# mahbhlddnhakkh/yuv-manipulations-2

Measured on AMD Instinct MI355X. Metric: megapixels/sec DCT compress+decompress, 4K IYUV; achieved HBM GB/s vs peak, higher is better.
Workload: dtype u8/int16 (fp32 transform)

## Files before the change

### yuv-manipulations-2_amd/csrc/k_huff_decode.hip

```cpp
#include "codec_common.hpp"
#include "coef_xform.h"
#include "downscale.h"
#include "huff_common.hpp"
#include "idct_scaled.h"
#include "jpeg_export.h"
#include "k1_store.hpp"
#include "k_metric.hpp"
#include "k_stream.hpp"
#include "requant.h"
#include "xform_common.hpp"

namespace myyuv_gpu {

namespace {

constexpr uint32_t kStageQuads = 320;
constexpr uint32_t kZeroBit = kStageQuads * 128u;
constexpr uint32_t kGposQuads = 8 * 64 * 4 / 16;

#ifndef MYYUV_K5_GROUP
#define MYYUV_K5_GROUP 2
#endif
#ifndef MYYUV_K5_FORMS
#define MYYUV_K5_FORMS 1
// ... 434 lines not shown

__global__ __launch_bounds__(64, MYYUV_K5_WAVES) void k_decode_idct(const uint8_t* __restrict__ in,
                                                   const uint32_t* __restrict__ in_size,
                                                   uint32_t cap,
                                                   const StreamDesc* __restrict__ desc,
                                                   const uint32_t* __restrict__ local_off,
                                                   const uint32_t* __restrict__ tile_pre,
                                                   FrameGeom G, uint32_t tiles_p0,
                                                   uint32_t tiles_p1, const QTables* __restrict__ qt,
                                                   uint4* __restrict__ coef,
                                                   uint8_t* __restrict__ frame,
                                                   unsigned long long* __restrict__ err) {
  static_assert(sizeof(uint4) * kStageQuads >= sizeof(float) * xf::kXfTile16, "the tile over the stage");
  __shared__ uint4 stq[kStageQuads + 1 + kGposQuads];
  __shared__ float sq[64];
  __shared__ uint16_t s_blk[64];
  const uint32_t lane = threadIdx.x;
  if (lane == 0) stq[kStageQuads] = make_uint4(0u, 0u, 0u, 0u);
  {
    const uint32_t t = blockIdx.x;
    const int p = t >= tiles_p0 ? (t >= tiles_p0 + tiles_p1 ? 2 : 1) : 0;
    __builtin_amdgcn_global_load_lds((const void*)&qt->q[p][lane], (__attribute__((address_space(3))) void*)sq, 4,
                                     0, 0);
  }
#ifdef MYYUV_STAMPS
  DStamps dst;
  DStamps* ds = &dst;
  dst.prev = __builtin_amdgcn_s_memtime();
#pragma unroll
  for (int k = 0; k < 8; k++) dst.acc[k] = k == 7 ? 1u : 0u;
#else
  DStamps* ds = nullptr;
#endif
  DecodeGroup D;
  uint32_t nw[32];
#pragma unroll
  for (int w = 0; w < 32; w++) nw[w] = 0;
  bool direct;
  if (!decode_group(in, in_size, cap, desc, local_off, tile_pre, G, tiles_p0, tiles_p1, coef, err, stq, D, nw,
                    direct, ds))
    return;
  DSTAMP(4);
  if (D.live && direct) {
#pragma unroll
    for (int c = 0; c < 8; c++) {
      const uint4 v = coef[coef_quad(D.gbase + D.g, c)];
      nw[4 * c] = v.x;
      nw[4 * c + 1] = v.y;
      nw[4 * c + 2] = v.z;
      nw[4 * c + 3] = v.w;
    }
  }
  const int p = D.p;
  xf::Unit U;
  U.p = p;
  U.cum = G.cum[p];
  U.nb = G.cum[p + 1] - G.cum[p];
  U.poff = p == 0 ? G.poff[0] : (p == 1 ? G.poff[1] : G.poff[2]);
  U.pw = p == 0 ? G.pw[0] : (p == 1 ? G.pw[1] : G.pw[2]);
  U.bw = p == 0 ? G.bw[0] : (p == 1 ? G.bw[1] : G.bw[2]);
  U.bmag = p == 0 ? G.bmag[0] : (p == 1 ? G.bmag[1] : G.bmag[2]);
  U.local0 = 0;
  uint8_t* fr = frame + (size_t)D.f * G.fbytes;
  uint32_t acc = nw[0] & 0xFFFF0000u;
#pragma unroll
  for (int w = 1; w < 32; w++) acc |= nw[w];
  const bool isdc = D.live && acc == 0u;
  if (isdc) {
    const uint32_t v4 = dc_block_pixels((int16_t)nw[0], sq[0]);
    const uint2 row = make_uint2(v4, v4);
#pragma unroll
    for (uint32_t r = 0; r < 8; r++) {
      const uint32_t off = xf::block_row_offset(U, D.g - U.cum, r);
      *reinterpret_cast<uint2*>(fr + off) = row;
    }
  }
  const uint64_t rest = __ballot(D.live && !isdc);
  const uint32_t nrest = (uint32_t)__popcll(rest);
  const uint32_t rrank = __builtin_amdgcn_mbcnt_hi((uint32_t)(rest >> 32), __builtin_amdgcn_mbcnt_lo((uint32_t)rest, 0u));
  if (D.live && !isdc) s_blk[rrank] = (uint16_t)lane;
  float* tile = reinterpret_cast<float*>(stq);
#pragma unroll 1
  for (uint32_t base = 0; base < nrest;) {
    const bool wide = nrest - base > 8u;
    const uint32_t span = wide ? 16u : 8u, stride = wide ? (uint32_t)xf::kTile : (uint32_t)xf::kTile8;
    const uint32_t s = rrank - base;
    if (D.live && !isdc && rrank >= base && s < span) {
      uint4* img = reinterpret_cast<uint4*>(tile + s * stride + (wide ? xf::img_word(s) : 0u));
#pragma unroll
      for (int c = 0; c < 8; c++) img[c] = make_uint4(nw[4 * c], nw[4 * c + 1], nw[4 * c + 2], nw[4 * c + 3]);
    }
    if (lane < span && base + lane >= nrest) {
      uint4* img = reinterpret_cast<uint4*>(tile + lane * stride + (wide ? xf::img_word(lane) : 0u));
#pragma unroll
      for (int c = 0; c < 8; c++) img[c] = make_uint4(0u, 0u, 0u, 0u);
    }
    xf::wave_sync();
    if (wide) {
      const uint32_t q = lane & 3u, b = lane >> 2;
      uint2 w0, w1;
      xf::idct_rows(tile + b * xf::kTile, q, b, sq, w0, w1);
      if (base + b < nrest) {
        const uint32_t gl = D.g0 + s_blk[base + b];
        const uint32_t off = xf::block_row_offset(U, gl - U.cum, 2u * q);
        *reinterpret_cast<uint2*>(fr + off) = w0;
        *reinterpret_cast<uint2*>(fr + off + U.pw) = w1;
      }
    } else {
      const uint32_t r = lane & 7u, b = lane >> 3;
      float qc[8];
#pragma unroll
      for (int k = 0; k < 8; k++) qc[k] = sq[8 * k + r];
      const uint2 w = xf::idct_row8(tile + b * xf::kTile8, r, qc);
      if (base + b < nrest) {
        const uint32_t gl = D.g0 + s_blk[base + b];
        *reinterpret_cast<uint2*>(fr + xf::block_row_offset(U, gl - U.cum, r)) = w;
      }
    }
    xf::wave_sync();
    base += span;
  }
  DSTAMP(5);
#ifdef MYYUV_STAMPS
  const uint32_t wid = blockIdx.y * gridDim.x + blockIdx.x;
#pragma unroll
  for (int k = 0; k < 8; k++)
    if (lane == (uint32_t)k && wid < 65536) g_dec_wstamps[wid * 8 + k] = dst.acc[k];
#endif
}

constexpr uint32_t kSpanStageQuads = 288;
constexpr uint32_t kSpanZeroBit = kSpanStageQuads * 128u;
constexpr uint32_t kSpanGroups = kDecSpan / kWave;
static_assert(sizeof(uint4) * kSpanStageQuads >= sizeof(float) * xf::kXfTile16, "the tile over the stage");
static_assert(16 * (kSpanStageQuads - 1) >= 15 + 255, "a round holds its first chunk wherever it starts in its quad");
#if MYYUV_DEC_SPAN <= 256
typedef uint32_t SpanEnt;
__device__ __forceinline__ SpanEnt span_ent(uint32_t idx, uint32_t off, uint32_t s) {
  return (off & 0xFFFFu) | (s << 16) | (idx << 24);
}
__device__ __forceinline__ uint32_t ent_off(SpanEnt e) { return e & 0xFFFFu; }
__device__ __forceinline__ uint32_t ent_size(SpanEnt e) { return (e >> 16) & 0xFFu; }
__device__ __forceinline__ uint32_t ent_idx(SpanEnt e) { return e >> 24; }
#else
typedef uint2 SpanEnt;
__device__ __forceinline__ SpanEnt span_ent(uint32_t idx, uint32_t off, uint32_t s) {
  return make_uint2(off, s | (idx << 8));
}
__device__ __forceinline__ uint32_t ent_off(SpanEnt e) { return e.x; }
__device__ __forceinline__ uint32_t ent_size(SpanEnt e) { return e.y & 0xFFu; }
__device__ __forceinline__ uint32_t ent_idx(SpanEnt e) { return e.y >> 8; }
#endif

__global__ __launch_bounds__(64, MYYUV_K5_WAVES) void k_decode_span(const uint8_t* __restrict__ in,
                                                   const uint32_t* __restrict__ in_size,
                                                   uint32_t cap,
                                                   const StreamDesc* __restrict__ desc,
                                                   const uint32_t* __restrict__ local_off,
                                                   const uint32_t* __restrict__ tile_pre,
                                                   FrameGeom G, uint32_t spans_p0,
                                                   uint32_t spans_p1, const QTables* __restrict__ qt,
                                                   uint4* __restrict__ coef,
                                                   uint8_t* __restrict__ frame,
                                                   unsigned long long* __restrict__ err) {
  __shared__ uint4 stq[kSpanStageQuads + 1 + kGposQuads];
  __shared__ float sq[64];
  __shared__ uint16_t s_blk[64];
  __shared__ SpanEnt s_ent[kDecSpan];
  const uint32_t lane = threadIdx.x;
  if (lane == 0) stq[kSpanStageQuads] = make_uint4(0u, 0u, 0u, 0u);
  const uint32_t t = blockIdx.x;
  const int p = t >= spans_p0 ? (t >= spans_p0 + spans_p1 ? 2 : 1) : 0;
  __builtin_amdgcn_global_load_lds((const void*)&qt->q[p][lane], (__attribute__((address_space(3))) void*)sq, 4, 0,
                                   0);
  const uint32_t f = blockIdx.y;
  const uint32_t nblk = G.cum[3];
  const uint32_t gbase = f * nblk;
  const uint32_t ntiles = (nblk + kScanTile - 1) / kScanTile;
  in += (size_t)f * cap;
  desc += f;
  local_off += gbase;
  tile_pre += (size_t)f * (ntiles + 1);
  auto sel3 = [p](uint32_t a0, uint32_t a1, uint32_t a2) { return p == 0 ? a0 : (p == 1 ? a1 : a2); };
  const uint32_t cum_p = sel3(G.cum[0], G.cum[1], G.cum[2]), cum_p1 = sel3(G.cum[1], G.cum[2], G.cum[3]);
  const uint32_t span_in_plane = t - sel3(0u, spans_p0, spans_p0 + spans_p1);
  const uint32_t b0 = cum_p + span_in_plane * kDecSpan;
  const uint32_t b1 = min(b0 + kDecSpan, cum_p1);
  const StreamDesc dsc = *desc;
  const uint32_t isz = in_size[f];
  const uint32_t b1c = min(b1, nblk - 1);
  const uint32_t lo_p = local_off[cum_p], tp_p = tile_pre[cum_p / kScanTile];
  uint32_t lo_j[kSpanGroups], tp_j[kSpanGroups];
#pragma unroll
  for (uint32_t j = 0; j < kSpanGroups; j++) {
    const uint32_t gs = b0 + kWave * j < b1 ? b0 + kWave * j : b0;
    lo_j[j] = local_off[gs];
    tp_j[j] = tile_pre[gs / kScanTile];
  }
  const uint32_t lo_1 = local_off[b1c], tp_1 = tile_pre[b1c / kScanTile];
  const uint32_t stot = tile_pre[ntiles];
  __builtin_amdgcn_sched_barrier(0);
  if (dsc.bad != 0) {
    asm volatile("s_waitcnt vmcnt(0)" ::: "memory");
    return;
  }
  const uint32_t plane_pre = lo_p + tp_p;
  const uint32_t limit = min(isz, cap);
  const uint32_t end_scan = b1 == nblk ? stot : lo_1 + tp_1;
  const uint32_t cpos = sel3(dsc.content_pos[0], dsc.content_pos[1], dsc.content_pos[2]);
  const uint32_t csize = sel3(dsc.content_size[0], dsc.content_size[1], dsc.content_size[2]);
  const uint32_t spos = sel3(dsc.sizes_pos[0], dsc.sizes_pos[1], dsc.sizes_pos[2]);
  const uint32_t E_span = cpos + min(end_scan - plane_pre, csize);
  const uint32_t pre0 = lo_j[0] + tp_j[0] - plane_pre;

  xf::Unit U;
  U.p = p;
  U.cum = cum_p;
  U.nb = cum_p1 - cum_p;
  U.poff = sel3(G.poff[0], G.poff[1], G.poff[2]);
  U.pw = sel3(G.pw[0], G.pw[1], G.pw[2]);
  U.bw = sel3(G.bw[0], G.bw[1], G.bw[2]);
  U.bmag = p == 0 ? G.bmag[0] : (p == 1 ? G.bmag[1] : G.bmag[2]);
  U.local0 = 0;
  uint8_t* fr = frame + (size_t)f * G.fbytes;

  uint32_t sz[kSpanGroups], rel[kSpanGroups];
  bool ok[kSpanGroups];
#pragma unroll
  for (uint32_t j = 0; j < kSpanGroups; j++) {
    const uint32_t g = b0 + kWave * j + lane;
    sz[j] = in[spos + ((g < b1 ? g : b1 - 1) - cum_p)];
  }
  bool over = false;
#pragma unroll
  for (uint32_t j = 0; j < kSpanGroups; j++) {
    const bool live = b0 + kWave * j + lane < b1;
    const uint32_t s = live ? sz[j] : 0u;
    rel[j] = lo_j[j] + tp_j[j] - plane_pre + wave_incl_scan(s) - s;
    ok[j] = live && rel[j] + s <= csize;
    over = over || (live && !ok[j]);
  }
  if (over) record_error(err, 2ull * ((uint64_t)G.fbase * nblk + gbase + cum_p), 9 );
  uint32_t hw[kSpanGroups], tw[kSpanGroups];
  bool cand[kSpanGroups];
#pragma unroll
  for (uint32_t j = 0; j < kSpanGroups; j++) {
    cand[j] = ok[j] && sz[j] == kSingleChunk && cpos + rel[j] + kSingleChunk <= limit;
    const uint8_t* a = in + (cand[j] ? cpos + rel[j] : 0u);
    __builtin_memcpy(&hw[j], a, 4);
    __builtin_memcpy(&tw[j], a + 3, 4);
  }
  asm volatile("s_waitcnt vmcnt(0)" ::: "memory");
  const float q0 = sq[0];
  uint32_t nreal = 0;
#pragma unroll
  for (uint32_t j = 0; j < kSpanGroups; j++) {
    uint32_t key;
    const bool single = single_chunk_key(hw[j], tw[j], key) && cand[j];
    if (single) {
      const uint32_t v4 = dc_block_pixels((int16_t)(((int32_t)(key << 21)) >> 21), q0);
      const uint2 row = make_uint2(v4, v4);
      const uint32_t local = b0 + kWave * j + lane - cum_p;
#pragma unroll
      for (uint32_t r = 0; r < 8; r++) *reinterpret_cast<uint2*>(fr + xf::block_row_offset(U, local, r)) = row;
    }
    const bool real = ok[j] && !single;
    const uint64_t m = __ballot(real);
    const uint32_t rank =
        nreal + __builtin_amdgcn_mbcnt_hi((uint32_t)(m >> 32), __builtin_amdgcn_mbcnt_lo((uint32_t)m, 0u));
    if (real) s_ent[rank] = span_ent(kWave * j + lane, rel[j] - pre0, sz[j]);
    nreal += (uint32_t)__popcll(m);
  }
  xf::wave_sync();

  float* tile = reinterpret_cast<float*>(stq);
  const uint32_t npass = (nreal + kWave - 1) / kWave;
#pragma unroll 1
  for (uint32_t pass = 0; pass < npass; pass++) {
    uint32_t ones = ~0u;
    asm volatile("" : "+s"(ones));
    const uint32_t lane = __builtin_amdgcn_mbcnt_hi(ones, __builtin_amdgcn_mbcnt_lo(ones, 0u));
    uint32_t* gcol = reinterpret_cast<uint32_t*>(stq + kSpanStageQuads + 1) + lane;
    const uint32_t e0 = kWave * pass, nhere = min(nreal - e0, (uint32_t)kWave);
    const bool have = lane < nhere;
    const SpanEnt ent = s_ent[e0 + (have ? lane : nhere - 1u)];
    const uint32_t s = have ? ent_size(ent) : 0u;
    const uint32_t prel = pre0 + ent_off(ent);
    const uint32_t g = b0 + ent_idx(ent);
    const uint32_t first = (uint32_t)__builtin_amdgcn_readfirstlane((int)prel);
    const uint32_t E = min(E_span, cpos + (uint32_t)__builtin_amdgcn_readlane((int)(prel + ent_size(ent)), 63));
    auto window = [&](uint32_t A, uint32_t& aw, uint32_t& wend, uint32_t& nq, uint32_t& nfull) {
      aw = A & ~15u;
      wend = aw + 16 * (kSpanStageQuads - 1);
      nq = E > aw ? (min(E, wend) - aw + 15) >> 4 : 0u;
      nfull = limit >= aw ? min(nq, (limit - aw) >> 4) : 0u;
    };
    auto load4 = [&](uint32_t aw, uint32_t nfull) {
#pragma unroll
      for (int m = 0; m < 4; m++) {
        const uint32_t o = nfull > 0 ? aw + 16 * min(lane + 64u * m, nfull - 1) : 0u;
        __builtin_amdgcn_global_load_lds((const void*)(in + o),
                                         (__attribute__((address_space(3))) void*)(stq + 64 * m), 16, 0, 0);
      }
    };
    uint32_t aw, wend, nq, nfull;
    window(cpos + first, aw, wend, nq, nfull);
    __syncthreads();
    load4(aw, nfull);
    auto stage = [&]() {
      asm volatile("s_waitcnt vmcnt(0)" ::: "memory");
      for (uint32_t k = lane + 256; k < nfull; k += 64)
        stq[k] = *reinterpret_cast<const uint4*>(in + aw + 16 * k);
      for (uint32_t k = nfull + lane; k <= nq; k += 64) {
        uint32_t v[4] = {0, 0, 0, 0};
        if (k < nq) {
#pragma unroll
          for (uint32_t b = 0; b < 16; b++) {
            const uint32_t a = aw + 16 * k + b;
            if (a < limit) v[b >> 2] |= (uint32_t)in[a] << (8 * (b & 3));
          }
        }
        stq[k] = make_uint4(v[0], v[1], v[2], v[3]);
      }
      __syncthreads();
    };
    uint32_t nw[32];
#pragma unroll
    for (int w = 0; w < 32; w++) nw[w] = 0;
    int code = 0;
    bool direct = false;
    uint64_t pending = __ballot(have);
    stage();
    while (pending) {
      const bool mine = ((pending >> lane) & 1) && cpos + prel + s <= wend;
      const LdsChunk lc{reinterpret_cast<const uint32_t*>(stq), mine ? cpos + prel - aw : 0u};
      Table T;
      const int pcode = parse_table(lc, mine ? s : 0u, T, gcol);
      const bool go = mine && pcode == 0;
      int dcode = 0;
      const bool failed = decode_regular<kSpanZeroBit>(lc, T, gcol, go && T.regular, nw);
      if (go && (!T.regular || failed)) {
        direct = true;
        dcode = decode_general(lc, T, coef, gbase + g);
      }
      if (mine) code = go ? dcode : pcode;
      pending &= ~__ballot(mine);
      if (pending) {
        __syncthreads();
        const int lo = __ffsll((long long)pending) - 1;
        window(cpos + (uint32_t)__builtin_amdgcn_readlane((int)prel, lo), aw, wend, nq, nfull);
        load4(aw, nfull);
        stage();
      }
    }
    if (have && code) record_error(err, 2ull * ((uint64_t)G.fbase * nblk + gbase + g) + 1, code);
    if (have && direct) {
#pragma unroll
      for (int c = 0; c < 8; c++) {
        const uint4 v = coef[coef_quad(gbase + g, c)];
        nw[4 * c] = v.x;
        nw[4 * c + 1] = v.y;
        nw[4 * c + 2] = v.z;
        nw[4 * c + 3] = v.w;
      }
    }
    uint32_t acc = nw[0] & 0xFFFF0000u;
#pragma unroll
    for (int w = 1; w < 32; w++) acc |= nw[w];
    const bool isdc = have && acc == 0u;
    if (isdc) {
      const uint32_t v4 = dc_block_pixels((int16_t)nw[0], sq[0]);
      const uint2 row = make_uint2(v4, v4);
#pragma unroll
      for (uint32_t r = 0; r < 8; r++) *reinterpret_cast<uint2*>(fr + xf::block_row_offset(U, g - cum_p, r)) = row;
    }
    const uint64_t rest = __ballot(have && !isdc);
    const uint32_t nrest = (uint32_t)__popcll(rest);
    const uint32_t rrank =
        __builtin_amdgcn_mbcnt_hi((uint32_t)(rest >> 32), __builtin_amdgcn_mbcnt_lo((uint32_t)rest, 0u));
    if (have && !isdc) s_blk[rrank] = (uint16_t)ent_idx(ent);
#pragma unroll 1
    for (uint32_t base = 0; base < nrest;) {
      const bool wide = nrest - base > 8u;
      const uint32_t span = wide ? 16u : 8u, stride = wide ? (uint32_t)xf::kTile : (uint32_t)xf::kTile8;
      const uint32_t sl = rrank - base;
      if (have && !isdc && rrank >= base && sl < span) {
        uint4* img = reinterpret_cast<uint4*>(tile + sl * stride + (wide ? xf::img_word(sl) : 0u));
#pragma unroll
        for (int c = 0; c < 8; c++) img[c] = make_uint4(nw[4 * c], nw[4 * c + 1], nw[4 * c + 2], nw[4 * c + 3]);
      }
      if (lane < span && base + lane >= nrest) {
        uint4* img = reinterpret_cast<uint4*>(tile + lane * stride + (wide ? xf::img_word(lane) : 0u));
#pragma unroll
        for (int c = 0; c < 8; c++) img[c] = make_uint4(0u, 0u, 0u, 0u);
      }
      xf::wave_sync();
      if (wide) {
        const uint32_t q = lane & 3u, b = lane >> 2;
        uint2 w0, w1;
        xf::idct_rows(tile + b * xf::kTile, q, b, sq, w0, w1);
        if (base + b < nrest) {
          const uint32_t off = xf::block_row_offset(U, b0 - cum_p + s_blk[base + b], 2u * q);
          *reinterpret_cast<uint2*>(fr + off) = w0;
          *reinterpret_cast<uint2*>(fr + off + U.pw) = w1;
        }
      } else {
        const uint32_t r = lane & 7u, b = lane >> 3;
        float qc[8];
#pragma unroll
        for (int k = 0; k < 8; k++) qc[k] = sq[8 * k + r];
        const uint2 w = xf::idct_row8(tile + b * xf::kTile8, r, qc);
        if (base + b < nrest)
          *reinterpret_cast<uint2*>(fr + xf::block_row_offset(U, b0 - cum_p + s_blk[base + b], r)) = w;
      }
      xf::wave_sync();
      base += span;
    }
  }
}

struct DecodeRun {
  uint32_t f;
  int p;
  uint32_t jo0, n;
  bool live;
};
__device__ __forceinline__ bool decode_run_at(const uint8_t* __restrict__ in, const uint32_t* __restrict__ in_size,
                                              uint32_t cap, const StreamDesc* __restrict__ desc,
                                              const uint32_t* __restrict__ local_off,
                                              const uint32_t* __restrict__ tile_pre, const FrameGeom& G,
                                              unsigned long long* __restrict__ err, uint4* stq, const int p,
                                              const uint32_t j, const uint32_t n, uint32_t (&nw)[32], bool& live_out,
                                              bool& good) {
  const uint32_t f = blockIdx.y;
  const uint32_t nblk = G.cum[3];
  const uint32_t gbase = f * nblk;
  const uint32_t ntiles = (nblk + kScanTile - 1) / kScanTile;
  in += (size_t)f * cap;
  desc += f;
  local_off += gbase;
  tile_pre += (size_t)f * (ntiles + 1);
  const uint32_t lane = threadIdx.x;
  uint32_t* gtab = reinterpret_cast<uint32_t*>(stq + kStageQuads + 1);
  uint32_t* gcol = gtab + lane;
  auto sel3 = [p](uint32_t a0, uint32_t a1, uint32_t a2) { return p == 0 ? a0 : (p == 1 ? a1 : a2); };
  const uint32_t cum_p = sel3(G.cum[0], G.cum[1], G.cum[2]);
  const uint32_t jg = j & ~(uint32_t)(kWave - 1), npre = j - jg;
  const bool live = lane < n;
  const uint32_t g = cum_p + j + lane;
  const StreamDesc dsc = *desc;
  const uint32_t isz = in_size[f];
  const uint32_t lo_p = local_off[cum_p], tp_p = tile_pre[cum_p / kScanTile];
  const uint32_t lo_g = local_off[cum_p + jg], tp_g = tile_pre[(cum_p + jg) / kScanTile];
  __builtin_amdgcn_sched_barrier(0);
  const bool bad = dsc.bad != 0;
  const uint32_t limit = bad ? 0u : min(isz, cap);
  const uint32_t cpos = sel3(dsc.content_pos[0], dsc.content_pos[1], dsc.content_pos[2]);
  const uint32_t csize = sel3(dsc.content_size[0], dsc.content_size[1], dsc.content_size[2]);
  const uint32_t spos = sel3(dsc.sizes_pos[0], dsc.sizes_pos[1], dsc.sizes_pos[2]);
  const uint32_t s = in[bad ? 0u : spos + j + (live ? lane : n - 1u)];
  const uint32_t sp = in[bad ? 0u : spos + jg + (lane < npre ? lane : 0u)];
  const uint32_t incl = wave_incl_scan(live ? s : 0u);
  const uint32_t pincl = wave_incl_scan(lane < npre ? sp : 0u);
  const uint32_t total = (uint32_t)__builtin_amdgcn_readlane((int)incl, 63);
  const uint32_t pre0 = (lo_g + tp_g) - (lo_p + tp_p) + (uint32_t)__builtin_amdgcn_readlane((int)pincl, 63);
  const uint32_t rel = pre0 + incl - (live ? s : 0u);
  const uint32_t E = cpos + min(pre0 + total, csize);
  auto window = [&](uint32_t A, uint32_t& aw, uint32_t& wend, uint32_t& nq, uint32_t& nfull) {
    aw = A & ~15u;
    wend = aw + 16 * (kStageQuads - 1);
    nq = E > aw ? (min(E, wend) - aw + 15) >> 4 : 0u;
    nfull = limit >= aw ? min(nq, (limit - aw) >> 4) : 0u;
  };
  auto load4 = [&](uint32_t aw, uint32_t nfull) {
#pragma unroll
    for (int m = 0; m < 4; m++) {
      const uint8_t* src = nfull > 0 ? in + aw + 16 * min(lane + 64u * m, nfull - 1) : in;
      __builtin_amdgcn_global_load_lds((const void*)src, (__attribute__((address_space(3))) void*)(stq + 64 * m),
                                       16, 0, 0);
    }
  };
  uint32_t aw, wend, nq, nfull;
  window(cpos + pre0, aw, wend, nq, nfull);
  load4(aw, nfull);

  bool ok = live && !bad;
  if (ok && rel + s > csize) {
    record_error(err, 2ull * ((uint64_t)G.fbase * nblk + gbase + cum_p), 9 );
    ok = false;
  }

  int code = 0;
  uint64_t pending = __ballot(ok);
  auto stage = [&]() {
    asm volatile("s_waitcnt vmcnt(0)" ::: "memory");
    for (uint32_t q = lane + 256; q < nfull; q += 64)
      stq[q] = *reinterpret_cast<const uint4*>(in + aw + 16 * q);
    for (uint32_t q = nfull + lane; q <= nq; q += 64) {
      uint32_t v[4] = {0, 0, 0, 0};
      if (q < nq) {
#pragma unroll
        for (uint32_t b = 0; b < 16; b++) {
          const uint32_t a = aw + 16 * q + b;
          if (a < limit) v[b >> 2] |= (uint32_t)in[a] << (8 * (b & 3));
        }
      }
      stq[q] = make_uint4(v[0], v[1], v[2], v[3]);
    }
    __syncthreads();
  };
  if (pending) stage();
  while (pending) {
    const bool mine = ((pending >> lane) & 1) && cpos + rel + s <= wend;
    const LdsChunk lc{reinterpret_cast<const uint32_t*>(stq), mine ? cpos + rel - aw : 0u};
    Table T;
    const int pcode = parse_table(lc, mine ? s : 0u, T, gcol);
    const bool go = mine && pcode == 0;
    int dcode = 0;
    const bool failed = decode_regular(lc, T, gcol, go && T.regular, nw);
    uint64_t dm = __ballot(go && (!T.regular || failed));
    while (dm) {
      const uint32_t rk = __builtin_amdgcn_mbcnt_hi((uint32_t)(dm >> 32), __builtin_amdgcn_mbcnt_lo((uint32_t)dm, 0u));
      const bool sel = ((dm >> lane) & 1) && rk < 16u;
      if (sel) {
        uint16_t* slot = reinterpret_cast<uint16_t*>(gtab) + 64u * rk;
        dcode = decode_general_to(lc, T, [=](uint32_t z, uint16_t v) { slot[z] = v; });
        const uint4* img = reinterpret_cast<const uint4*>(slot);
#pragma unroll
        for (int c = 0; c < 8; c++) {
          const uint4 v = img[c];
          nw[4 * c] = v.x;
          nw[4 * c + 1] = v.y;
          nw[4 * c + 2] = v.z;
          nw[4 * c + 3] = v.w;
        }
// ... 887 lines not shown
```

### yuv-manipulations-2_amd/csrc/xform_common.hpp

```cpp
#pragma once
#include <stddef.h>

#include "codec_common.hpp"
#include "fdct_bfly.h"

namespace myyuv_gpu {
namespace xf {

constexpr float c_dct[64] = MYYUV_DCT_MATRIX;
constexpr int kTile = 72;
constexpr int kXfTile16 = 16 * kTile;
constexpr float kMagic = 0x1.8p23f;
constexpr float kMagicPx = 0x1.8p23f + 128.0f;
constexpr float kHalfDown = 0x1.fffffep-2f;

__device__ __forceinline__ constexpr int tix(int i, int j) { return (i >> 1) * 18 + 2 * j + (i & 1); }

__device__ __forceinline__ uint32_t bits(float x) { return __builtin_bit_cast(uint32_t, x); }

__device__ __forceinline__ void wave_sync() {
  __builtin_amdgcn_fence(__ATOMIC_RELEASE, "wavefront");
  __builtin_amdgcn_wave_barrier();
  __builtin_amdgcn_fence(__ATOMIC_ACQUIRE, "wavefront");
}

template <int kCtrl>
__device__ __forceinline__ uint32_t quad_perm(uint32_t v) {
  return (uint32_t)__builtin_amdgcn_update_dpp((int)v, (int)v, kCtrl, 0xF, 0xF, false);
}
__device__ __forceinline__ uint32_t quad_xor1(uint32_t v) { return quad_perm<0xB1>(v); }
__device__ __forceinline__ uint32_t quad_xor2(uint32_t v) { return quad_perm<0x4E>(v); }
__device__ __forceinline__ uint32_t quad_lane0(uint32_t v) { return quad_perm<0x00>(v); }

__device__ __forceinline__ void fence16(float (&a)[16]) {
  asm volatile("" : "+v"(a[0]), "+v"(a[1]), "+v"(a[2]), "+v"(a[3]), "+v"(a[4]), "+v"(a[5]),
               "+v"(a[6]), "+v"(a[7]), "+v"(a[8]), "+v"(a[9]), "+v"(a[10]), "+v"(a[11]),
               "+v"(a[12]), "+v"(a[13]), "+v"(a[14]), "+v"(a[15]));
}

struct Unit {
  int p;
  uint32_t local0;
  uint32_t nb;
  uint32_t cum;
  uint32_t poff;
  uint32_t pw;
  uint32_t bw;
  uint64_t bmag;
};

template <class T>
__device__ __forceinline__ T pick(bool p1, bool p2, T a0, T a1, T a2) {
  return p2 ? a2 : (p1 ? a1 : a0);
}

__device__ __forceinline__ Unit unit_of(const FrameGeom& G, uint32_t u) {
  const bool p1 = u >= G.ucum[1], p2 = u >= G.ucum[2];
  Unit r;
  r.p = p2 ? 2 : (p1 ? 1 : 0);
  r.local0 = (u - pick(p1, p2, G.ucum[0], G.ucum[1], G.ucum[2])) * kXfUnit;
  r.cum = pick(p1, p2, G.cum[0], G.cum[1], G.cum[2]);
  r.nb = pick(p1, p2, G.cum[1], G.cum[2], G.cum[3]) - r.cum;
  r.poff = pick(p1, p2, G.poff[0], G.poff[1], G.poff[2]);
  r.pw = pick(p1, p2, G.pw[0], G.pw[1], G.pw[2]);
  r.bw = pick(p1, p2, G.bw[0], G.bw[1], G.bw[2]);
  r.bmag = pick(p1, p2, G.bmag[0], G.bmag[1], G.bmag[2]);
  return r;
}

__device__ __forceinline__ uint32_t block_row_offset(const Unit& U, uint32_t local, uint32_t r) {
  uint32_t by = local;
  if (U.bmag != 0) {
    const uint64_t lo = (uint64_t)local * (uint32_t)U.bmag;
    const uint64_t hi = (uint64_t)local * (uint32_t)(U.bmag >> 32) + (lo >> 32);
    by = (uint32_t)(hi >> 32);
  }
  const uint32_t bx = local - by * U.bw;
  return U.poff + (by * 8u + r) * U.pw + bx * 8u;
}

__device__ __forceinline__ uint32_t first_unit() {
  return __builtin_amdgcn_readfirstlane(blockIdx.x * 4u + (threadIdx.x >> 6));
}
__device__ __forceinline__ uint32_t unit_stride() { return gridDim.x * 4u; }

constexpr int kAlwaysSteps = 3;
template <bool kInverse, bool kSkip = false, bool kFence = true>
__device__ __forceinline__ void dot_rows(const float (&P)[16], float (&out)[16]) {
  if (kSkip) {
#pragma unroll
    for (int j = 0; j < 16; j++) out[j] = 0.0f;
  }
#pragma unroll
  for (int k = 0; k < 8; k++) {
    if (kSkip && (kFence || k >= kAlwaysSteps) && !__any(P[2 * k] != 0.0f || P[2 * k + 1] != 0.0f)) continue;
    float pr[16];
#pragma unroll
    for (int v = 0; v < 8; v++) {
      const float d = c_dct[kInverse ? k * 8 + v : v * 8 + k];
      pr[2 * v] = P[2 * k] * d;
      pr[2 * v + 1] = P[2 * k + 1] * d;
    }
#pragma unroll
    for (int j = 0; j < 16; j++) out[j] = (k == 0 && !kSkip) ? pr[j] : out[j] + pr[j];
    if (kFence) fence16(out);
  }
}

__device__ __forceinline__ void transpose_tile(float* tb, uint32_t q, const float (&M)[16],
                                               float (&P)[16]) {
#pragma unroll
  for (int i = 0; i < 8; i++) {
    tb[tix(i, 2 * q)] = M[2 * i];
    tb[tix(i, 2 * q + 1)] = M[2 * i + 1];
  }
  wave_sync();
#pragma unroll
  for (int k = 0; k < 8; k++) {
    const float2 v = *reinterpret_cast<const float2*>(tb + tix(2 * q, k));
    P[2 * k] = v.x;
    P[2 * k + 1] = v.y;
  }
}

__device__ __forceinline__ constexpr int tixf(int i, int j) { return (i & 3) * 18 + 2 * j + (i >> 2); }

__device__ __forceinline__ void transpose_fwd(float* tb, uint32_t q, const float (&M)[16], float (&P)[16]) {
#pragma unroll
  for (int i = 0; i < 8; i++) {
    tb[tixf(i, 2 * q)] = M[2 * i];
    tb[tixf(i, 2 * q + 1)] = M[2 * i + 1];
  }
  wave_sync();
#pragma unroll
  for (int k = 0; k < 8; k++) {
    const float2 v = *reinterpret_cast<const float2*>(tb + tixf(q, k));
    P[2 * k] = v.x;
    P[2 * k + 1] = v.y;
  }
}

__device__ __forceinline__ float sbyte(uint32_t w, int k) {
  return (float)(int)(int8_t)(uint8_t)(w >> (8 * k));
}

__device__ __forceinline__ uint4 load_rows(const uint8_t* __restrict__ frame, const FrameGeom& G,
                                           uint32_t ua, uint32_t b, uint32_t q) {
  const uint32_t f = div_magic(ua, G.umag);
  const Unit U = unit_of(G, ua - f * G.ucum[3]);
  const uint32_t local = U.local0 + b;
  const uint32_t off = block_row_offset(U, local < U.nb ? local : U.nb - 1, 2u * q);
  const uint8_t* fr = frame + (size_t)f * G.fbytes;
  const uint2 r0 = *reinterpret_cast<const uint2*>(fr + off);
  const uint2 r1 = *reinterpret_cast<const uint2*>(fr + off + U.pw);
  return make_uint4(r0.x, r0.y, r1.x, r1.y);
}

// ... 40 lines not shown

template <bool kZero>
struct HiZero {
  static constexpr bool value = kZero;
};

__device__ __forceinline__ void fdct_load(const uint8_t* img, uint32_t q, uint32_t (&xr)[4]) {
#pragma unroll
  for (int m = 0; m < 4; m++)
    xr[m] = *reinterpret_cast<const uint16_t*>(img + 16 * m + 2 * q) |
            ((uint32_t)*reinterpret_cast<const uint16_t*>(img + 16 * m + 8 + 2 * q) << 16);
  wave_sync();
}

constexpr int kSqR = 3 * 64, kSqKb = 2 * 3 * 64, kSqWords = 2 * 3 * 64 + 3 * 8;

template <bool kPerBlock, class Emit>
__device__ __forceinline__ uint64_t fdct_fast(const uint32_t (&xr)[4], float* tb, uint32_t q, bool live,
                                              const float* sqr, int p, Emit&& emit) {
  uint32_t a = 0;
#pragma unroll
  for (int m = 0; m < 4; m++) a = __builtin_amdgcn_sad_u8(xr[m], 0x80808080u, a);
  a += quad_xor1(a);
  a += quad_xor2(a);
  float T[16];
#pragma unroll
  for (int c = 0; c < 2; c++) {
    float px[8], t[8];
#pragma unroll
    for (int m = 0; m < 8; m++) px[m] = (float)((xr[m >> 1] >> (8 * (2 * (m & 1) + c))) & 0xFFu);
    myyuv_bfly::bfly_cols(px, t);
#pragma unroll
    for (int i = 0; i < 8; i++) T[2 * i + c] = t[i];
  }
  float P[16];
  transpose_fwd(tb, q, T, P);
  const float af = (float)a;
  const float* Rq = sqr + kSqR + p * 64 + 8u * q;
  const float* kb = sqr + kSqKb + p * 8 + q;
  uint32_t c[16];
  auto row = [&](auto hc) {
    constexpr int h = decltype(hc)::value ? 1 : 0;
    float x[8], y[8];
#pragma unroll
    for (int k = 0; k < 8; k++) x[k] = P[2 * k + h];
    myyuv_bfly::bfly_rows(x, y);
    float em = 0.0f;
#pragma unroll
    for (int v = 0; v < 8; v++) {
      const float t = y[v] * Rq[32 * h + v];
      const float u = t + kMagic;
      const float e = t - (u - kMagic);
      em = __builtin_fmaxf(em, __builtin_fabsf(e));
      c[2 * v + h] = bits(u);
    }
    return __builtin_fmaf(af, kb[4 * h], em);
  };
  auto finish = [&](float mx, auto hz) -> uint64_t {
    const uint64_t bad = __builtin_amdgcn_ballot_w64(mx >= 0.5f);
    if (bad == 0) {
      emit(c, true, hz);
      return 0;
    }
    if (!kPerBlock) return bad;
    uint32_t fb = mx >= 0.5f ? 1u : 0u;
    fb |= quad_xor1(fb);
    fb |= quad_xor2(fb);
    emit(c, fb == 0u, hz);
    return __builtin_amdgcn_ballot_w64(fb != 0u);
  };
  bool skip = false;
  const float kb4 = __builtin_bit_cast(float, __builtin_amdgcn_readfirstlane(bits(sqr[kSqKb + p * 8 + 4])));
  if (myyuv_bfly::bfly_zero_rows_tested(kb4)) {
    float x1[8];
#pragma unroll
    for (int k = 0; k < 8; k++) x1[k] = P[2 * k + 1];
    const bool zr = myyuv_bfly::bfly_zero_row(x1, af, kb[4]) || !live;
    skip = __builtin_amdgcn_ballot_w64(zr) == ~0ull;
  }
  const float m0 = row(HiZero<false>{});
  if (skip) {
#pragma unroll
    for (int v = 0; v < 8; v++) c[2 * v + 1] = 0u;
    return finish(m0, HiZero<true>{});
  }
  return finish(__builtin_fmaxf(m0, row(HiZero<true>{})), HiZero<false>{});
}

template <class Emit>
__device__ __forceinline__ void fdct_exact(const uint32_t (&xr)[4], float* tb, uint32_t q, const float* sqr, int p,
                                           Emit&& emit) {
  const uint32_t n0 = 8u * q;
  float T[16];
  fdct_stage1_exact(xr, T);
  float P[16];
  transpose_fwd(tb, q, T, P);
  float Y[16];
  dot_rows<false>(P, Y);
  const float4* R4 = reinterpret_cast<const float4*>(sqr + kSqR + p * 64 + n0);
  const float4 r0 = R4[0], r1 = R4[1], r2 = R4[8], r3 = R4[9];
  const float rr[16] = {r0.x, r2.x, r0.y, r2.y, r0.z, r2.z, r0.w, r2.w,
                        r1.x, r3.x, r1.y, r3.y, r1.z, r3.z, r1.w, r3.w};
  uint32_t c[16];
  float mx = 0.0f;
#pragma unroll
  for (int j = 0; j < 16; j++) {
    const float tq = Y[j] * rr[j];
    const float uu = tq + kMagic;
    const float e = tq - (uu - kMagic);
    mx = __builtin_fmaxf(mx, __builtin_fmaf(__builtin_fabsf(tq), kNearRel, __builtin_fabsf(e)));
    c[j] = bits(uu);
  }
  if (mx >= 0.5f) {
    const float* Qt = sqr + p * 64 + n0;
#pragma unroll
    for (int j = 0; j < 16; j++) c[j] = (uint32_t)(int)roundf(Y[j] / Qt[(j >> 1) + 32 * (j & 1)]);
  }
  emit(c);
}

template <class Emit>
__device__ __forceinline__ void fdct_core(const uint8_t* img, float* tb, uint32_t q, bool live, const float* sqr,
                                          int p, Emit&& emit) {
  uint32_t xr[4];
  fdct_load(img, q, xr);
  if (__builtin_expect(fdct_fast<false>(xr, tb, q, live, sqr, p, emit) != 0, 0)) {
    wave_sync();
    fdct_exact(xr, tb, q, sqr, p, [&](const uint32_t (&c)[16]) { emit(c, true, HiZero<false>{}); });
  }
}

template <bool kHiZero = false>
__device__ __forceinline__ void pack_quads(const uint32_t (&c)[16], uint32_t q, uint4& lo, uint4& hi,
                                           uint32_t& rm) {
  lo.x = __builtin_amdgcn_perm(c[2], c[0], 0x05040100u);
  lo.y = __builtin_amdgcn_perm(c[6], c[4], 0x05040100u);
  lo.z = __builtin_amdgcn_perm(c[10], c[8], 0x05040100u);
  lo.w = __builtin_amdgcn_perm(c[14], c[12], 0x05040100u);
  hi = make_uint4(0, 0, 0, 0);
  if (!kHiZero) {
    hi.x = __builtin_amdgcn_perm(c[3], c[1], 0x05040100u);
    hi.y = __builtin_amdgcn_perm(c[7], c[5], 0x05040100u);
    hi.z = __builtin_amdgcn_perm(c[11], c[9], 0x05040100u);
    hi.w = __builtin_amdgcn_perm(c[15], c[13], 0x05040100u);
  }
  const bool nzl = (lo.x | lo.y | lo.z | lo.w) != 0u, nzh = !kHiZero && (hi.x | hi.y | hi.z | hi.w) != 0u;
  rm = (nzl ? 1u << q : 0u) | (nzh ? 16u << q : 0u);
  rm |= quad_xor1(rm);
  rm |= quad_xor2(rm);
}

__device__ __forceinline__ constexpr uint32_t img_word(uint32_t b) { return 4u * ((b >> 2) & 1u); }

__device__ __forceinline__ void idct_rows(float* tb, uint32_t q, uint32_t b, const float* Qt, uint2& w0,
                                          uint2& w1) {
  const uint32_t* tw = reinterpret_cast<const uint32_t*>(tb) + img_word(b);
  uint32_t zc[8];
#pragma unroll
  for (int k = 0; k < 8; k++) zc[k] = tw[k * 4 + q];
  wave_sync();
  float qk[16];
#pragma unroll
  for (int k = 0; k < 8; k++) {
    const float2 v = *reinterpret_cast<const float2*>(Qt + k * 8 + 2 * q);
    qk[2 * k] = v.x;
    qk[2 * k + 1] = v.y;
  }

  float Um[16];
#pragma unroll
  for (int j = 0; j < 16; j++) Um[j] = 0.0f;
#pragma unroll
  for (int k = 0; k < 8; k++) {
    if (k >= kAlwaysSteps && !__any(zc[k] != 0u)) continue;
    const float z0 = (float)(int16_t)zc[k] * qk[2 * k];
    const float z1 = (float)(int16_t)(zc[k] >> 16) * qk[2 * k + 1];
    float pr[16];
#pragma unroll
    for (int i = 0; i < 8; i++) {
      pr[2 * i] = c_dct[k * 8 + i] * z0;
      pr[2 * i + 1] = c_dct[k * 8 + i] * z1;
    }
#pragma unroll
    for (int j = 0; j < 16; j++) Um[j] = Um[j] + pr[j];
  }

  float P[16];
  transpose_tile(tb, q, Um, P);

  float S[16];
  dot_rows<true, true, false>(P, S);
  uint32_t px[16];
  bool tie = false;
#pragma unroll
  for (int j = 0; j < 16; j++) {
    S[j] = __builtin_amdgcn_fmed3f(S[j], -128.0f, 127.0f);
    const float uu = S[j] + kMagicPx;
    tie = tie || __builtin_amdgcn_fractf(S[j]) == 0.5f;
    px[j] = bits(uu);
  }
  if (tie) {
#pragma unroll
    for (int j = 0; j < 16; j++)
      px[j] = (uint32_t)((int)__builtin_truncf(S[j] + __builtin_copysignf(kHalfDown, S[j])) + 128);
  }
  w0 = make_uint2(__builtin_amdgcn_perm(__builtin_amdgcn_perm(px[6], px[4], 0x0c0c0400u),
                                                    __builtin_amdgcn_perm(px[2], px[0], 0x0c0c0400u),
                                                    0x05040100u),
                              __builtin_amdgcn_perm(__builtin_amdgcn_perm(px[14], px[12], 0x0c0c0400u),
                                                    __builtin_amdgcn_perm(px[10], px[8], 0x0c0c0400u),
                                                    0x05040100u));
  w1 = make_uint2(__builtin_amdgcn_perm(__builtin_amdgcn_perm(px[7], px[5], 0x0c0c0400u),
                                                    __builtin_amdgcn_perm(px[3], px[1], 0x0c0c0400u),
                                                    0x05040100u),
                              __builtin_amdgcn_perm(__builtin_amdgcn_perm(px[15], px[13], 0x0c0c0400u),
                                                    __builtin_amdgcn_perm(px[11], px[9], 0x0c0c0400u),
                                                    0x05040100u));
}

constexpr int kTile8 = 72;
#ifndef MYYUV_ALWAYS8
#define MYYUV_ALWAYS8 2
#endif
constexpr int kAlways8 = MYYUV_ALWAYS8;
__device__ __forceinline__ uint2 idct_row8(float* tb, uint32_t r, const float (&qc)[8]) {
  const int16_t* im = reinterpret_cast<const int16_t*>(tb);
  int zk[8];
#pragma unroll
  for (int k = 0; k < 8; k++) zk[k] = im[8 * k + r];
  wave_sync();
  float Um[8];
#pragma unroll
  for (int i = 0; i < 8; i++) Um[i] = 0.0f;
#pragma unroll
  for (int k = 0; k < 8; k++) {
    if (k >= kAlways8 && !__any(zk[k] != 0)) continue;
    const float z = (float)zk[k] * qc[k];
#pragma unroll
    for (int i = 0; i < 8; i++) Um[i] = Um[i] + c_dct[k * 8 + i] * z;
  }
#pragma unroll
  for (int i = 0; i < 8; i++) tb[8 * i + r] = Um[i];
  wave_sync();
  const float4 p0 = *reinterpret_cast<const float4*>(tb + 8 * r);
  const float4 p1 = *reinterpret_cast<const float4*>(tb + 8 * r + 4);
  const float P[8] = {p0.x, p0.y, p0.z, p0.w, p1.x, p1.y, p1.z, p1.w};
  float S[8];
#pragma unroll
  for (int v = 0; v < 8; v++) S[v] = 0.0f;
#pragma unroll
  for (int k = 0; k < 8; k++) {
    if (k >= kAlways8 && !__any(P[k] != 0.0f)) continue;
#pragma unroll
    for (int v = 0; v < 8; v++) S[v] = S[v] + P[k] * c_dct[k * 8 + v];
  }
  uint32_t px[8];
  bool tie = false;
#pragma unroll
  for (int v = 0; v < 8; v++) {
    S[v] = __builtin_amdgcn_fmed3f(S[v], -128.0f, 127.0f);
    tie = tie || __builtin_amdgcn_fractf(S[v]) == 0.5f;
    px[v] = bits(S[v] + kMagicPx);
  }
  if (tie) {
#pragma unroll
    for (int v = 0; v < 8; v++)
      px[v] = (uint32_t)((int)__builtin_truncf(S[v] + __builtin_copysignf(kHalfDown, S[v])) + 128);
  }
  return make_uint2(__builtin_amdgcn_perm(__builtin_amdgcn_perm(px[3], px[2], 0x0c0c0400u),
                                          __builtin_amdgcn_perm(px[1], px[0], 0x0c0c0400u), 0x05040100u),
                    __builtin_amdgcn_perm(__builtin_amdgcn_perm(px[7], px[6], 0x0c0c0400u),
                                          __builtin_amdgcn_perm(px[5], px[4], 0x0c0c0400u), 0x05040100u));
}

}
}
```

Before: 400,300.

## Add low-frequency corner IDCT fast path for blocks with only top-left coefficients

Classifies decoded non-DC blocks whose nonzero coefficients all lie in the top-left NxN corner (default 3x3) and runs a reduced IDCT for them, packing 16 blocks per wave with four lanes per block. The aim is to skip most of the full 8x8 separable transform, shared-tile staging and transposes for the many low-frequency blocks. Remaining blocks still take the general tiled path. The pixel rounding and packing code is factored into a shared host/device helper, and the block index array is narrowed to bytes. It adds an extra ballot, classification logic and another loop, and loads basis rows into shared memory.

```diff
diff --git a/yuv-manipulations-2_amd/csrc/k_huff_decode.hip b/yuv-manipulations-2_amd/csrc/k_huff_decode.hip
--- a/yuv-manipulations-2_amd/csrc/k_huff_decode.hip
+++ b/yuv-manipulations-2_amd/csrc/k_huff_decode.hip
@@ -610,6 +610,25 @@
 __device__ __forceinline__ uint32_t ent_idx(SpanEnt e) { return e.y >> 8; }
 #endif
 
+#ifndef MYYUV_CORNER_N
+#define MYYUV_CORNER_N 3
+#endif
+constexpr int kCornerN = MYYUV_CORNER_N;
+static_assert(kCornerN == 2 || kCornerN == 3, "the staged basis rows are 1 and 2");
+static_assert(xf::c_dct[0] == xf::c_dct[1] && xf::c_dct[0] == xf::c_dct[2] && xf::c_dct[0] == xf::c_dct[3] &&
+                  xf::c_dct[0] == xf::c_dct[4] && xf::c_dct[0] == xf::c_dct[5] && xf::c_dct[0] == xf::c_dct[6] &&
+                  xf::c_dct[0] == xf::c_dct[7],
+              "row 0 of the basis is one value: a corner lane's d[0], d[1]");
+constexpr uint32_t kCornerSlot = 6;
+__device__ const float d_corner_basis[16] = {
+    xf::c_dct[8],  xf::c_dct[9],  xf::c_dct[10], xf::c_dct[11], xf::c_dct[12], xf::c_dct[13], xf::c_dct[14], xf::c_dct[15],
+    xf::c_dct[16], xf::c_dct[17], xf::c_dct[18], xf::c_dct[19], xf::c_dct[20], xf::c_dct[21], xf::c_dct[22], xf::c_dct[23]};
+#if MYYUV_DEC_SPAN <= 256
+typedef uint8_t SpanIdx;
+#else
+typedef uint16_t SpanIdx;
+#endif
+
 __global__ __launch_bounds__(64, MYYUV_K5_WAVES) void k_decode_span(const uint8_t* __restrict__ in,
                                                    const uint32_t* __restrict__ in_size,
                                                    uint32_t cap,
@@ -623,7 +642,8 @@
                                                    unsigned long long* __restrict__ err) {
   __shared__ uint4 stq[kSpanStageQuads + 1 + kGposQuads];
   __shared__ float sq[64];
-  __shared__ uint16_t s_blk[64];
+  __shared__ SpanIdx s_blk[64];
+  __shared__ __attribute__((aligned(16))) float s_cd[16];
   __shared__ SpanEnt s_ent[kDecSpan];
   const uint32_t lane = threadIdx.x;
   if (lane == 0) stq[kSpanStageQuads] = make_uint4(0u, 0u, 0u, 0u);
@@ -631,6 +651,7 @@
   const int p = t >= spans_p0 ? (t >= spans_p0 + spans_p1 ? 2 : 1) : 0;
   __builtin_amdgcn_global_load_lds((const void*)&qt->q[p][lane], (__attribute__((address_space(3))) void*)sq, 4, 0,
                                    0);
+  const float cdv = d_corner_basis[lane & 15u];
   const uint32_t f = blockIdx.y;
   const uint32_t nblk = G.cum[3];
   const uint32_t gbase = f * nblk;
@@ -709,6 +730,7 @@
     __builtin_memcpy(&tw[j], a + 3, 4);
   }
   asm volatile("s_waitcnt vmcnt(0)" ::: "memory");
+  if (lane < 16u) s_cd[lane] = cdv;
   const float q0 = sq[0];
   uint32_t nreal = 0;
 #pragma unroll
@@ -822,23 +844,74 @@
         nw[4 * c + 3] = v.w;
       }
     }
-    uint32_t acc = nw[0] & 0xFFFF0000u;
-#pragma unroll
-    for (int w = 1; w < 32; w++) acc |= nw[w];
-    const bool isdc = have && acc == 0u;
+    uint32_t outc = 0u, edge = 0u, inc = nw[0] & 0xFFFF0000u;
+#pragma unroll
+    for (int w = 0; w < 32; w++) {
+      const int r = w >> 2, c0 = 2 * (w & 3);
+      if (r >= kCornerN || c0 >= kCornerN) {
+        outc |= nw[w];
+      } else {
+        if (c0 + 1 == kCornerN) edge |= nw[w];
+        if (w != 0) inc |= nw[w];
+      }
+    }
+    outc |= edge & 0xFFFF0000u;
+    const bool isdc = have && (outc | inc) == 0u;
     if (isdc) {
       const uint32_t v4 = dc_block_pixels((int16_t)nw[0], sq[0]);
       const uint2 row = make_uint2(v4, v4);
 #pragma unroll
       for (uint32_t r = 0; r < 8; r++) *reinterpret_cast<uint2*>(fr + xf::block_row_offset(U, g - cum_p, r)) = row;
     }
-    const uint64_t rest = __ballot(have && !isdc);
-    const uint32_t nrest = (uint32_t)__popcll(rest);
-    const uint32_t rrank =
-        __builtin_amdgcn_mbcnt_hi((uint32_t)(rest >> 32), __builtin_amdgcn_mbcnt_lo((uint32_t)rest, 0u));
-    if (have && !isdc) s_blk[rrank] = (uint16_t)ent_idx(ent);
+    const bool corner = have && !isdc && outc == 0u;
+    const uint64_t mcor = __ballot(corner), mgen = __ballot(have && !isdc && !corner);
+    const uint32_t nc = (uint32_t)__popcll(mcor);
+    const uint32_t nrest = nc + (uint32_t)__popcll(mgen);
+    const uint32_t ncu = (nc + 7u) >> 4;
+    const uint32_t ncc = min(nc, 16u * ncu);
+    const uint64_t mine_m = corner ? mcor : mgen;
+    const uint32_t rrank = (corner ? 0u : nc) + __builtin_amdgcn_mbcnt_hi((uint32_t)(mine_m >> 32),
+                                                                         __builtin_amdgcn_mbcnt_lo((uint32_t)mine_m, 0u));
+    if (have && !isdc) s_blk[rrank] = (SpanIdx)ent_idx(ent);
 #pragma unroll 1
-    for (uint32_t base = 0; base < nrest;) {
+    for (uint32_t cb = 0; cb < ncc; cb += 16u) {
+      uint32_t* cw = reinterpret_cast<uint32_t*>(tile);
+      const uint32_t sl = rrank - cb;
+      if (corner && rrank >= cb && sl < 16u) {
+#pragma unroll
+        for (int r = 0; r < kCornerN; r++)
+          *reinterpret_cast<uint2*>(cw + sl * kCornerSlot + 2 * r) = make_uint2(nw[4 * r], nw[4 * r + 1]);
+      }
+      xf::wave_sync();
+      const uint32_t q = lane & 3u, b = lane >> 2;
+      const uint32_t bs = min(b, ncc - cb - 1u);
+      int z[kCornerN * kCornerN];
+#pragma unroll
+      for (int r = 0; r < kCornerN; r++) {
+        const uint2 v = *reinterpret_cast<const uint2*>(cw + bs * kCornerSlot + 2 * r);
+        z[r * kCornerN] = (int16_t)v.x;
+        z[r * kCornerN + 1] = (int16_t)(v.x >> 16);
+        if (kCornerN > 2) z[r * kCornerN + 2] = (int16_t)v.y;
+      }
+      float d[2 * kCornerN];
+      d[0] = d[1] = xf::c_dct[0];
+#pragma unroll
+      for (int k = 1; k < kCornerN; k++) {
+        const float2 v = *reinterpret_cast<const float2*>(s_cd + 8 * (k - 1) + 2 * q);
+        d[2 * k] = v.x;
+        d[2 * k + 1] = v.y;
+      }
+      uint2 w0, w1;
+      xf::idct_corner<kCornerN>(z, sq, d, w0, w1);
+      if (cb + b < ncc) {
+        const uint32_t off = xf::block_row_offset(U, b0 - cum_p + s_blk[cb + b], 2u * q);
+        *reinterpret_cast<uint2*>(fr + off) = w0;
+        *reinterpret_cast<uint2*>(fr + off + U.pw) = w1;
+      }
+      xf::wave_sync();
+    }
+#pragma unroll 1
+    for (uint32_t base = ncc; base < nrest;) {
       const bool wide = nrest - base > 8u;
       const uint32_t span = wide ? 16u : 8u, stride = wide ? (uint32_t)xf::kTile : (uint32_t)xf::kTile8;
       const uint32_t sl = rrank - base;
diff --git a/yuv-manipulations-2_amd/csrc/xform_common.hpp b/yuv-manipulations-2_amd/csrc/xform_common.hpp
--- a/yuv-manipulations-2_amd/csrc/xform_common.hpp
+++ b/yuv-manipulations-2_amd/csrc/xform_common.hpp
@@ -3,6 +3,8 @@
 
 #include "codec_common.hpp"
 #include "fdct_bfly.h"
+
+#define MYYUV_IDCT_HD __host__ __device__ __forceinline__
 
 namespace myyuv_gpu {
 namespace xf {
@@ -349,6 +351,50 @@
 
 __device__ __forceinline__ constexpr uint32_t img_word(uint32_t b) { return 4u * ((b >> 2) & 1u); }
 
+MYYUV_IDCT_HD float px_clamp(float s) {
+#if defined(__HIP_DEVICE_COMPILE__)
+  return __builtin_amdgcn_fmed3f(s, -128.0f, 127.0f);
+#else
+  return s < -128.0f ? -128.0f : (s > 127.0f ? 127.0f : s);
+#endif
+}
+MYYUV_IDCT_HD float px_fract(float s) {
+#if defined(__HIP_DEVICE_COMPILE__)
+  return __builtin_amdgcn_fractf(s);
+#else
+  return s - __builtin_floorf(s);
+#endif
+}
+MYYUV_IDCT_HD uint32_t px_pack4(uint32_t a, uint32_t b, uint32_t c, uint32_t d) {
+#if defined(__HIP_DEVICE_COMPILE__)
+  return __builtin_amdgcn_perm(__builtin_amdgcn_perm(d, c, 0x0c0c0400u), __builtin_amdgcn_perm(b, a, 0x0c0c0400u),
+                               0x05040100u);
+#else
+  return (a & 0xFFu) | ((b & 0xFFu) << 8) | ((c & 0xFFu) << 16) | ((d & 0xFFu) << 24);
+#endif
+}
+MYYUV_IDCT_HD bool pixel_rows(float (&S)[16], uint2& w0, uint2& w1) {
+  uint32_t px[16];
+  bool tie = false;
+#pragma unroll
+  for (int j = 0; j < 16; j++) {
+    S[j] = px_clamp(S[j]);
+    const float uu = S[j] + kMagicPx;
+    tie = tie || px_fract(S[j]) == 0.5f;
+    px[j] = __builtin_bit_cast(uint32_t, uu);
+  }
+  if (tie) {
+#pragma unroll
+    for (int j = 0; j < 16; j++)
+      px[j] = (uint32_t)((int)__builtin_truncf(S[j] + __builtin_copysignf(kHalfDown, S[j])) + 128);
+  }
+  w0.x = px_pack4(px[0], px[2], px[4], px[6]);
+  w0.y = px_pack4(px[8], px[10], px[12], px[14]);
+  w1.x = px_pack4(px[1], px[3], px[5], px[7]);
+  w1.y = px_pack4(px[9], px[11], px[13], px[15]);
+  return tie;
+}
+
 __device__ __forceinline__ void idct_rows(float* tb, uint32_t q, uint32_t b, const float* Qt, uint2& w0,
                                           uint2& w1) {
   const uint32_t* tw = reinterpret_cast<const uint32_t*>(tb) + img_word(b);
@@ -387,32 +433,41 @@
 
   float S[16];
   dot_rows<true, true, false>(P, S);
-  uint32_t px[16];
-  bool tie = false;
-#pragma unroll
-  for (int j = 0; j < 16; j++) {
-    S[j] = __builtin_amdgcn_fmed3f(S[j], -128.0f, 127.0f);
-    const float uu = S[j] + kMagicPx;
-    tie = tie || __builtin_amdgcn_fractf(S[j]) == 0.5f;
-    px[j] = bits(uu);
-  }
-  if (tie) {
-#pragma unroll
-    for (int j = 0; j < 16; j++)
-      px[j] = (uint32_t)((int)__builtin_truncf(S[j] + __builtin_copysignf(kHalfDown, S[j])) + 128);
-  }
-  w0 = make_uint2(__builtin_amdgcn_perm(__builtin_amdgcn_perm(px[6], px[4], 0x0c0c0400u),
-                                                    __builtin_amdgcn_perm(px[2], px[0], 0x0c0c0400u),
-                                                    0x05040100u),
-                              __builtin_amdgcn_perm(__builtin_amdgcn_perm(px[14], px[12], 0x0c0c0400u),
-                                                    __builtin_amdgcn_perm(px[10], px[8], 0x0c0c0400u),
-                                                    0x05040100u));
-  w1 = make_uint2(__builtin_amdgcn_perm(__builtin_amdgcn_perm(px[7], px[5], 0x0c0c0400u),
-                                                    __builtin_amdgcn_perm(px[3], px[1], 0x0c0c0400u),
-                                                    0x05040100u),
-                              __builtin_amdgcn_perm(__builtin_amdgcn_perm(px[15], px[13], 0x0c0c0400u),
-                                                    __builtin_amdgcn_perm(px[11], px[9], 0x0c0c0400u),
-                                                    0x05040100u));
+  pixel_rows(S, w0, w1);
+}
+
+template <int N>
+MYYUV_IDCT_HD bool idct_corner(const int (&z)[N * N], const float* Qt, const float (&d)[2 * N], uint2& w0, uint2& w1) {
+  static_assert(N >= 2 && N <= 4, "the corner classes: 2x2, 3x3, 4x4");
+  float Z[N * N];
+#pragma unroll
+  for (int k = 0; k < N; k++) {
+#pragma unroll
+    for (int j = 0; j < N; j++) Z[k * N + j] = (float)z[k * N + j] * Qt[k * 8 + j];
+  }
+  float Uq[2 * N];
+#pragma unroll
+  for (int j = 0; j < N; j++) {
+#pragma unroll
+    for (int h = 0; h < 2; h++) {
+      float a = d[h] * Z[j];
+#pragma unroll
+      for (int k = 1; k < N; k++) a = a + d[2 * k + h] * Z[k * N + j];
+      Uq[2 * j + h] = a;
+    }
+  }
+  float S[16];
+#pragma unroll
+  for (int v = 0; v < 8; v++) {
+#pragma unroll
+    for (int h = 0; h < 2; h++) {
+      float a = Uq[h] * c_dct[v];
+#pragma unroll
+      for (int k = 1; k < N; k++) a = a + Uq[2 * k + h] * c_dct[k * 8 + v];
+      S[2 * v + h] = a;
+    }
+  }
+  return pixel_rows(S, w0, w1);
 }
 
 constexpr int kTile8 = 72;
```

Result: no change. 402,600 (median of 6 runs) (+0.6%).
